# heiheishuang/MuDG

Measured on AMD Instinct MI355X. Metric: DDIM denoise steps/sec, MDM1024 576x1024x16f (CFG: 2 UNet forwards + fused update per step, per clip), higher is better.
Workload: dtype bf16; 1 GPU; MDM1024 latents (B=1,4,16,72,128) + c_concat 8ch, context (B,333,1024), 50-step uniform_trailing DDIM schedule, cfg 7.5, guidance_rescale 0.7, eta 1.0, v-prediction, dynamic rescale; clips_per_gpu=1, parallelism=clip-DP x1 (no in-step collective), launch=hipGraph replay of each UNet pass (cond+uncond batched)

## Files before the change

include/mudg_hip.h:

```cpp
#ifndef MUDG_HIP_H
#define MUDG_HIP_H

#include <stdint.h>

#ifdef __cplusplus
extern "C" {
#endif

#define MUDG_OK          0
#define MUDG_EINVAL     -1
#define MUDG_ELAUNCH    -2
#define MUDG_EUNSUPPORTED -3

int mudg_version(void);
int mudg_operand_dtype(void);
const char* mudg_last_error(void);

typedef struct MudgGemmDesc {
    const void* X;
    const void* X2;
    const void* W;
    void*       Y;
    const float* bias;
    const float* gbias;
// ... 17 lines not shown
    float* stats;
    int subpixel;
    void* Y8; void* S8;
    int ldy8, lds8;
} MudgGemmDesc;
int mudg_gemm(const MudgGemmDesc* d, void* stream);
int mudg_gemm_stats_rows(const MudgGemmDesc* d);
int mudg_conv_subpixel_ok(const MudgGemmDesc* d);

typedef struct MudgAttnDesc {
    const void* Q; const void* K; const void* Vt; void* O;
    int F, heads, Nq, Nk;
    int ldq, ldk, ldvt, ldo;
    int64_t svt;
    int kv_div;
    float scale;
    int accumulate;
    const void* K2; const void* Vt2;
    int Nk2, ldk2, ldvt2, kv_div2;
    int64_t svt2;
    const void* Q8; const void* K8; const void* Qs; const void* Ks;
    int ldq8, ldk8, ldqs, ldks;
    int q_prescaled;
    float* Lse;
} MudgAttnDesc;
int mudg_attention(const MudgAttnDesc* d, void* stream);
int mudg_quantize_mxfp8(const void* X, int ldx, int64_t rows, int cols, void* Y8, int ldy, void* S, int lds, void* stream);

int mudg_temporal_attention(const void* QKV, void* O, int B, int T, int HW, int heads,
                            int ldqkv, int ldo, float scale, void* stream);
int mudg_temporal_self_attention_ok(int T, int HW, int heads, int C, int64_t ldx, int64_t ldw, int64_t ldo);
int mudg_temporal_self_attention(const void* X, const void* Wh, void* O, int B, int T, int HW, int heads, int C, int64_t ldx,
                                 int64_t ldw, int64_t ldo, float scale, void* stream);

int64_t mudg_groupnorm_ws_floats(int samples, int groups, int rows);
int mudg_groupnorm(const void* X, const void* X2, int csplit, int ldx, int ldx2, int x_fp32,
                   const float* gamma, const float* beta, void* Y, int ldy,
                   int samples, int rows, int C, int groups, float eps, int silu,
                   float* ws, void* stream);
int mudg_groupnorm_fused(const void* X, const void* X2, int csplit, int ldx, int ldx2, int x_fp32,
                         const float* gamma, const float* beta, void* Y, int ldy,
                         int samples, int rows, int C, int groups, float eps, int silu,
                         const float* P1, const float* P2, float* ws, void* stream);

int mudg_groupnorm_fused_rows(const void* X, const void* X2, int csplit, int ldx, int ldx2, int x_fp32,
                              const float* gamma, const float* beta, void* Y, int ldy,
                              int samples, int rows, int C, int groups, float eps, int silu,
                              const float* P1, int p1_rows, const float* P2, int p2_rows, float* ws, void* stream);

int mudg_layernorm(const void* X, int ldx, int x_fp32, const float* gamma, const float* beta,
                   void* Y, int ldy, int rows, int C, float eps, void* stream);

int mudg_softmax_rows(const float* S, int lds, void* P, int ldp, int rows, int cols, void* stream);

int mudg_timestep_embedding(const int64_t* t, const float* freqs, float* out, int n, int dim, void* stream);
int mudg_small_linear(const float* x, const void* W, int w_is_bf16, const float* b, float* y,
                      int M, int N, int K, int act_in, int act_out, int accumulate, void* stream);

int mudg_ncthw_to_rows(const void* src, int src_is_fp32, void* dst, int B, int C, int T, int HW,
                       int ld, int coff, int Ttot, int t0, void* stream);
int mudg_rows_to_ncthw(const void* src, int src_is_fp32, int ld, int coff, void* dst, int dst_is_fp32,
                       int B, int C, int T, int HW, float scale, int Ttot, int t0, void* stream);
int mudg_copy_rows(const void* src, int64_t lds, void* dst, int64_t ldd, int64_t rows, int64_t cols, void* stream);
int mudg_axpy_f32(float* y, const float* x, int64_t n, float alpha, void* stream);
int mudg_lincomb(float* out, const float* x, const float* y, const float* ca, const float* cb, int B, int64_t n,
                 void* stream);
// ... 182 lines not shown
```

mudg_amd/csrc/attention.hip:

```cpp
#include "attn_shared.h"
#include <cstdlib>

namespace {

#if MUDG_PLANES == 1
template <bool TWO>
__global__ __launch_bounds__(256, 2) void attn_kernel(const MudgAttnDesc p, const int nqt, const int total) {
    __shared__ __attribute__((aligned(16))) h16 Ks[2 * ATILE];
    __shared__ __attribute__((aligned(16))) h16 Vs[2 * ATILE];

    const int tid = threadIdx.x, lane = tid & 63, wave = tid >> 6;
    const int l31 = lane & 31, hi = lane >> 5;

    const int w = xcd_work_item(total);
    const int pair = w / nqt, qt = w - pair * nqt;
    const int f = pair / p.heads, h = pair - f * p.heads;
    const h16* Qp = reinterpret_cast<const h16*>(p.Q) + (int64_t)f * p.Nq * p.ldq + h * 64;
    h16* Op = reinterpret_cast<h16*>(p.O) + (int64_t)f * p.Nq * p.ldo + h * 64;

    const int q = qt * QB + wave * 32 + l31;
    const bool qok = q < p.Nq;

    h16x8 qf[1][4];
    load_q_frags(qf[0], Qp, q, p.ldq, 0, qok, hi);

    const int lrow = tid >> 3, kc = tid & 7;
    u32x4 kr[1][2], vr[1][2];

    f32x16 o[2], res[TWO ? 2 : 1];
    const float c = p.q_prescaled ? 1.0f : p.scale * 1.4426950408889634f;
    float inv = 0.f;
#pragma unroll
    for (int set = 0; set < (TWO ? 2 : 1); ++set) {
// ... 667 lines not shown
        __syncthreads();
    }

    char* mine = tsa_smem + wave * (2 * 3 * 2048);
#pragma unroll
    for (int pi = 0; pi < 2; ++pi) {
        char* qs = mine + pi * (3 * 2048);
#pragma unroll
        for (int nb = 0; nb < 12; ++nb) {
            Pack8 t;
#pragma unroll
            for (int i = 0; i < 4; ++i) t.h[i] = (h16)acc[pi][nb][i];
            const int u = 4 * (nb & 3) + g;
            const int off = (nb >> 2) == 2 ? c * 128 + ((u ^ tattn_fz(c >> 2)) << 3)
                                           : c * 128 + (((u >> 1) ^ (c & 7)) << 4) + ((u & 1) << 3);
            *reinterpret_cast<u32x2*>(qs + (nb >> 2) * 2048 + off) = t.u;
        }
    }
    __builtin_amdgcn_wave_barrier();
#pragma unroll
    for (int pi = 0; pi < 2; ++pi) {
        const char* qs = mine + pi * (3 * 2048);
        float ov[16];
        tattn_item_mfma(qs, qs + 2048, qs + 4096, c, g, 16, scale, ov);
        h16* dst = O + (row0 + (int64_t)c * HW + (2 * wave + pi)) * ldo + h * 64 + g * 8;
#pragma unroll
        for (int half = 0; half < 2; ++half) {
            h16x8 t;
#pragma unroll
            for (int e = 0; e < 8; ++e) t[e] = (h16)ov[half * 8 + e];
            st16(dst + half * 32, as_u32x4(t));
        }
    }
}
#endif

#if MUDG_PLANES > 1
template <bool TWO>
__global__ __launch_bounds__(256, PLANES == 2 ? 2 : 1) void attn_split_kernel(const MudgAttnDesc p, const int nqt, const int total) {
    extern __shared__ __attribute__((aligned(16))) char smem_raw[];
    h16* Ks = reinterpret_cast<h16*>(smem_raw);
    h16* Vs = Ks + 2 * PLANES * ATILE;

    const int tid = threadIdx.x, lane = tid & 63, wave = tid >> 6;
    const int l31 = lane & 31, hi = lane >> 5;
    const int w = xcd_work_item(total);
    const int pair = w / nqt, qt = w - pair * nqt;
    const int f = pair / p.heads, h = pair - f * p.heads;
    const int psq = p.ldq / PLANES, pso = p.ldo / PLANES;

    const h16* Qp = reinterpret_cast<const h16*>(p.Q) + (int64_t)f * p.Nq * p.ldq + h * 64;
    h16* Op = reinterpret_cast<h16*>(p.O) + (int64_t)f * p.Nq * p.ldo + h * 64;

    const int q = qt * QB + wave * 32 + l31;
    const bool qok = q < p.Nq;
    h16x8 qf[PLANES][4];
#pragma unroll
    for (int pl = 0; pl < PLANES; ++pl) load_q_frags(qf[pl], Qp, q, p.ldq, pl * psq, qok, hi);

    const int lrow = tid >> 3, kc = tid & 7;
    u32x4 kr[PLANES][2], vr[PLANES][2];

    f32x16 o[2], res[TWO ? 2 : 1];
    const float c = p.q_prescaled ? 1.0f : p.scale * 1.4426950408889634f;
#pragma unroll
    for (int set = 0; set < (TWO ? 2 : 1); ++set) {
// ... 575 lines not shown
           ldw >= C && ldo >= C;
#else
    (void)T; (void)HW; (void)heads; (void)C; (void)ldx; (void)ldw; (void)ldo;
    return 0;
#endif
}

extern "C" int mudg_temporal_self_attention(const void* X, const void* Wh, void* O, int B, int T, int HW, int heads, int C, int64_t ldx,
                                            int64_t ldw, int64_t ldo, float scale, void* stream) {
#if MUDG_PLANES == 1
    MUDG_REQUIRE(X && Wh && O, "mudg_temporal_self_attention: null pointer");
    MUDG_REQUIRE(B > 0, "mudg_temporal_self_attention: empty problem");
    MUDG_REQUIRE(aligned16(X) && aligned16(Wh) && aligned16(O), "mudg_temporal_self_attention: alignment");
    if (!mudg_temporal_self_attention_ok(T, HW, heads, C, ldx, ldw, ldo))
        MUDG_FAIL(MUDG_EUNSUPPORTED, "mudg_temporal_self_attention: T=%d HW=%d heads=%d C=%d outside the fused kernel (T = 16, HW %% 8 == 0, "
                  "C = 64 heads, dense 16-byte rows): project with mudg_gemm and call mudg_temporal_attention", T, HW, heads, C);
    const int64_t total = (int64_t)B * (HW / 8) * heads;
    MUDG_REQUIRE(total < (1ll << 31), "mudg_temporal_self_attention: grid too large");
    const int rc0 = mudg_lds_opt_in<tsattn_fused_kernel>(TSA_LDS, "mudg_temporal_self_attention");
    if (rc0 != MUDG_OK) return rc0;
    hipStream_t s = reinterpret_cast<hipStream_t>(stream);
    const int slot = mudg_prof_begin(MUDG_FAM_GEMM, s);
    hipLaunchKernelGGL(tsattn_fused_kernel, dim3((unsigned)total), dim3(256), TSA_LDS, s, (const h16*)X, (const h16*)Wh, (h16*)O, HW, heads, C,
                       ldx, ldw, ldo, scale, (int)total);
    const int rc = mudg_check_launch("mudg_temporal_self_attention");
    const double M = (double)B * T * HW;
    mudg_prof_end(slot, s, 2.0 * M * 3.0 * C * C + 4.0 * (double)B * HW * heads * T * T * 64.0, (2.0 * M * C + 3.0 * C * C) * 2.0);
    return rc;
#else
    (void)X; (void)Wh; (void)O; (void)B; (void)T; (void)HW; (void)heads; (void)C; (void)ldx; (void)ldw; (void)ldo; (void)scale; (void)stream;
    MUDG_FAIL(MUDG_EUNSUPPORTED, "mudg_temporal_self_attention: the fused kernel belongs to the 16-bit operand builds");
#endif
}
```

mudg_amd/csrc/attn_shared.h:

```cpp
#pragma once
#include "common.h"
#include <type_traits>

constexpr int QB = 128;
constexpr int KB = 64;
constexpr int ALD = 72;
constexpr int ATILE = 64 * ALD;

struct KvSet {
    const h16* Kp;
    const h16* Vp;
    int Nk, ldk, ldvt;
    int psk, psv;
};
__device__ __forceinline__ KvSet kv_set(const MudgAttnDesc& p, int f, int h, int set) {
    KvSet kv;
    if (set == 0) {
        kv.Kp = reinterpret_cast<const h16*>(p.K) + (int64_t)(f / p.kv_div) * p.Nk * p.ldk + h * 64;
        kv.Vp = reinterpret_cast<const h16*>(p.Vt) + (int64_t)(f / p.kv_div) * p.svt + (int64_t)(h * 64) * p.ldvt;
        kv.Nk = p.Nk; kv.ldk = p.ldk; kv.ldvt = p.ldvt;
    } else {
        kv.Kp = reinterpret_cast<const h16*>(p.K2) + (int64_t)(f / p.kv_div2) * p.Nk2 * p.ldk2 + h * 64;
        kv.Vp = reinterpret_cast<const h16*>(p.Vt2) + (int64_t)(f / p.kv_div2) * p.svt2 + (int64_t)(h * 64) * p.ldvt2;
        kv.Nk = p.Nk2; kv.ldk = p.ldk2; kv.ldvt = p.ldvt2;
// ... 188 lines not shown
        } else {
#pragma unroll
            for (int r = 0; r < 16; ++r) { o[0][r] = fmaf(o[0][r], inv, res[0][r]); o[1][r] = fmaf(o[1][r], inv, res[1][r]); }
            inv = 1.f;
        }
    }
    return inv;
}
__device__ __forceinline__ void finish_block16(const MudgAttnDesc& p, int f, int h, int q, bool qok, int hi, float c,
                                               float m_run, float l_run, const f32x16 (&o)[2], h16* Op) {
    const float l_tot = l_run + __shfl_xor(l_run, 32, 64);
    const float inv = 1.f / l_tot;
    store_lse(p, f, h, q, qok, hi, c, m_run, l_tot);
    if (qok) store_o16(o, inv, Op + (int64_t)q * p.ldo, hi, p.accumulate);
}

__device__ __forceinline__ __amdgpu_buffer_rsrc_t attn_rsrc(const h16* base) {
    return __builtin_amdgcn_make_buffer_rsrc(const_cast<h16*>(base), 0, (int)0x80000000u, 0x00020000);
}
typedef __attribute__((address_space(3))) void* attn_lptr_t;
__device__ __forceinline__ int swap_mid4(int row) {
    const int i16 = row & 15;
    return (row & ~15) | (i16 & 3) | ((i16 & 8) >> 1) | ((i16 & 4) << 1);
}
__device__ __forceinline__ void dma_offsets(int wave, int lane, int ldk, int ldvt, unsigned (&vk)[2], unsigned (&vv)[2]) {
#pragma unroll
    for (int i = 0; i < 2; ++i) {
        const int row = 16 * wave + 8 * i + (lane >> 3), slot = lane & 7;
        const int chunk = slot ^ ((row >> 1) & 7);
        vk[i] = (unsigned)swap_mid4(row) * (unsigned)ldk * 2u + (unsigned)chunk * 16u;
        vv[i] = (unsigned)row * (unsigned)ldvt * 2u + (unsigned)chunk * 16u;
    }
}
```

mudg_amd/engine/unet.py:

```python
import torch
import torch.nn as nn

from .. import ops
from . import packing as pk



import os as _os
_LEAN_ATTENTION = _os.environ.get("MUDG_ATTN_LEAN", "1") != "0"
_TCONV_SLAB = _os.environ.get("MUDG_TCONV_SLAB", "1") != "0"
_TSATTN_FUSED = _os.environ.get("MUDG_TSATTN_FUSED", "1") != "0"
_FP8_ATTENTION = _os.environ.get("MUDG_ATTN_FP8", "0") == "1"


class _Ctx:
    __slots__ = ("B", "T", "emb", "text", "img", "n_text", "n_img", "img_div", "kv_cache", "replicas", "skips")

    def __init__(self):
        self.replicas, self.skips = 1, None

    def fan_out(self, rows):
        r, self.replicas = self.replicas, 1
        self.B *= r
        self.emb = self.emb.repeat(r, 1)
        if self.skips is not None:
            self.skips[:] = [(ops.repeat_rows(t, r), h, w) for t, h, w in self.skips]
        return ops.repeat_rows(rows, r)


def _gn(mod, x, x2, samples, rows, silu):
    return ops.groupnorm(x, pk.f32(mod, "weight"), pk.f32(mod, "bias"), samples=samples, rows=rows, eps=mod.eps,
                         silu=silu, groups=mod.num_groups, x2=x2)


def _ln(mod, x):
    return ops.layernorm(x, pk.f32(mod, "weight"), pk.f32(mod, "bias"), eps=mod.eps)


def _linear(mod, x, residual=None, x2=None, stream=False, stats=False, hw=0):
    return ops.gemm(x, pk.linear(mod), bias=pk.f32(mod, "bias"), residual=residual, x2=x2, out_stream=stream, stats=stats, frame_rows=hw)


def _conv3x3(mod, x, frames, h, w, *, stride=1, upsample=False, gbias=None, rows_per_group=0, residual=None, x2=None,
             stream=False, stats=True, fp32=False):
    wmat, cpad, korder = pk.conv3x3(mod)
# ... 36 lines not shown
def temporal_conv_block(mod, x, ctx, hw):
    y = x
    stages = (mod.conv1, mod.conv2, mod.conv3, mod.conv4)
    for i, seq in enumerate(stages):
        norm, conv = seq[0], seq[-1]
        y = _gn(norm, y, None, ctx.B, ctx.T * hw, True)
        last = i == len(stages) - 1
        slab = (not last and _TCONV_SLAB and ops.tconv3_slab_ok(ctx.T, hw, conv.weight.shape[1])
                and not ops.tconv3_wide(ctx.T, hw, conv.weight.shape[1], conv.weight.shape[0]))
        y = ops.tconv3(y, pk.tconv(conv, slab), clips=ctx.B, t=ctx.T, hw=hw, cin=conv.weight.shape[1],
                       bias=pk.f32(conv, "bias"), residual=x if last else None, out_stream=last, stats=True, korder=int(slab))
    return y


def res_block(mod, x, x2, h, w, ctx):
    frames, hw = ctx.B * ctx.T, h * w
    a = _gn(mod.in_layers[0], x, x2, frames, hw, True)
    lin = mod.emb_layers[1]
    emb_out = ops.small_linear(ctx.emb, pk.f32(lin, "weight"), pk.f32(lin, "bias"), act_in=True)
    a = _conv3x3(mod.in_layers[2], a, frames, h, w, gbias=emb_out, rows_per_group=ctx.T * hw)
    a = _gn(mod.out_layers[0], a, None, frames, hw, True)
    if isinstance(mod.skip_connection, nn.Identity):
        if x2 is not None:
            raise RuntimeError("identity skip with a concatenated input")
        skip = x
    else:
        skip = _linear(mod.skip_connection, ops.cast_bf16(x), x2=None if x2 is None else ops.cast_bf16(x2), stream=True, hw=hw)
    out = _conv3x3(mod.out_layers[3], a, frames, h, w, residual=skip, stream=True)
    if mod.use_temporal_conv:
        out = temporal_conv_block(mod.temopral_conv, out, ctx, hw)
    return out


def _cross_kv(attn, ctx):
    k_text = ops.gemm(ctx.text, pk.linear(attn.to_k))
    vt_text, ld_text = _vt_projection(attn.to_v, ctx.text, ctx.B, ctx.n_text)
    if ctx.img is None or not attn.image_cross_attention:
        return k_text, vt_text, ld_text, None, None, 0
    k_img = ops.gemm(ctx.img, pk.linear(attn.to_k_ip))
    vt_img, ld_img = _vt_projection(attn.to_v_ip, ctx.img, ctx.img.shape[0] // ctx.n_img, ctx.n_img)
    return k_text, vt_text, ld_text, k_img, vt_img, ld_img


def spatial_block(blk, hcur, frames, hw, ctx, last):
    a1, a2 = blk.attn1, blk.attn2
    c, heads = hcur.shape[1], a1.heads
    n1 = _ln(blk.norm1, hcur)
    lean = _LEAN_ATTENTION and ops.hip.planes() <= 2
    wqk = pk.qk_prescaled(a1, a1.to_q, a1.to_k, a1.scale) if lean else pk.linear_cat(a1, "qk", (a1.to_q, a1.to_k))
    use_fp8 = lean and ops.hip.planes() == 1 and _FP8_ATTENTION and hw >= 512 and hw % 64 == 0
    fp8 = None
    if use_fp8:
        qk, q8, s8 = ops.gemm(n1, wqk, fp8=True)
        fp8 = (q8[:, :c], s8[:, :c // 32], q8[:, c:], s8[:, c // 32:])
    else:
        qk = ops.gemm(n1, wqk, frame_rows=hw)
    vt, ldv = _vt_projection(a1.to_v, n1, frames, hw)
    att = ops.empty_rows(frames * hw, c, ops.H16(), hcur.device)
    ops.attention(qk[:, :c], qk[:, c:], vt, att, frames=frames, heads=heads, nq=hw, nk=hw, ldvt=ldv, svt=c * ldv,
                  scale=a1.scale, q_prescaled=lean, fp8=fp8)
    hcur = _linear(a1.to_out[0], att, residual=hcur, stream=True, hw=hw)
    if ctx.replicas > 1:
        hcur = ctx.fan_out(hcur)
        frames = ctx.B * ctx.T
    n2 = _ln(blk.norm2, hcur)
    q2 = ops.gemm(n2, pk.linear(a2.to_q), frame_rows=hw)
    key = id(a2)
    if key not in ctx.kv_cache:
        ctx.kv_cache[key] = _cross_kv(a2, ctx)
    k_text, vt_text, ld_text, k_img, vt_img, ld_img = ctx.kv_cache[key]
    att2 = ops.empty_rows(frames * hw, c, ops.H16(), hcur.device)
    if k_img is not None and a2.image_cross_attention_scale != 1.0:
        raise NotImplementedError("image_cross_attention_scale != 1.0")
    ops.attention(q2, k_text, vt_text, att2, frames=frames, heads=heads, nq=hw, nk=ctx.n_text, ldvt=ld_text,
                  svt=c * ld_text, kv_div=ctx.T, scale=a2.scale, k2=k_img, vt2=vt_img, nk2=ctx.n_img,
                  ldvt2=ld_img if k_img is not None else None, svt2=c * ld_img if k_img is not None else None,
                  kv_div2=ctx.img_div)
    hcur = _linear(a2.to_out[0], att2, residual=hcur, stream=True, hw=hw)
    return _feed_forward(blk.ff, _ln(blk.norm3, hcur), hcur, stream=not last, hw=hw)


def spatial_transformer(mod, x, h, w, ctx):
    hw = h * w
    cur = _linear(mod.proj_in, _gn(mod.norm, x, None, ctx.B * ctx.T, hw, False), stream=True, hw=hw)
    n = len(mod.transformer_blocks)
    for i, blk in enumerate(mod.transformer_blocks):
        shared = ctx.replicas
        cur = spatial_block(blk, cur, ctx.B * ctx.T, hw, ctx, i == n - 1)
        if ctx.replicas != shared:
            x = ops.repeat_rows(x, shared)
    return _linear(mod.proj_out, cur, residual=x, stream=True, stats=True, hw=hw)


_TSATTN_MAX_C = 640


def _tsattn_fused(t, hw, heads, c, x, out):
    return (_TSATTN_FUSED and c == heads * 64 and c <= _TSATTN_MAX_C
            and ops.temporal_self_attention_ok(t, hw, heads, c, x.stride(0), c, out.stride(0)))


def temporal_block(blk, hcur, hw, ctx, last):
    for attn, norm in ((blk.attn1, blk.norm1), (blk.attn2, blk.norm2)):
        c = hcur.shape[1]
        n = _ln(norm, hcur)
        att = ops.empty_rows(hcur.shape[0], c, ops.H16(), hcur.device)
# ... 240 lines not shown
```

mudg_amd/hip.py:

```python
from __future__ import annotations

import ctypes as C
import os

_HERE = os.path.dirname(os.path.abspath(__file__))
LIB_PATHS = {"bf16": os.path.join(_HERE, "libmudg_hip.so"), "fp16": os.path.join(_HERE, "libmudg_hip_fp16.so"),
             "bf16x3": os.path.join(_HERE, "libmudg_hip_x3.so"), "bf16x6": os.path.join(_HERE, "libmudg_hip_x6.so")}
_MODES = {"bf16": (0, 1), "fp16": (1, 1), "bf16x3": (2, 2), "bf16x6": (3, 3)}
_operand = os.environ.get("MUDG_OPERAND", "bf16").lower()
LIB_PATH = LIB_PATHS["bf16"]


def set_operand(name: str) -> None:
    global _operand
    name = name.lower()
    if name not in LIB_PATHS:
        raise MudgError(f"unknown operand type {name!r} ({' | '.join(LIB_PATHS)})")
    if _lib is not None and name != _operand:
        raise MudgError("the operand type must be chosen before the first kernel call")
    _operand = name


def operand_name() -> str:
    return _operand
# ... 67 lines not shown
class WgradDesc(C.Structure):
    _fields_ = [
        ("A", C.c_void_p), ("B", C.c_void_p), ("out", C.c_void_p),
        ("lda", C.c_int64), ("ldb", C.c_int64), ("P", C.c_int64),
        ("M", C.c_int), ("C", C.c_int), ("taps", C.c_int), ("mode", C.c_int),
        ("Hin", C.c_int), ("Win", C.c_int), ("Hout", C.c_int), ("Wout", C.c_int), ("stride", C.c_int), ("pad", C.c_int),
        ("T", C.c_int), ("HW", C.c_int),
        ("slices", C.c_int), ("chunk", C.c_int64),
    ]


class ShortAttnDesc(C.Structure):
    _fields_ = [
        ("QKV", C.c_void_p), ("O", C.c_void_p),
        ("B", C.c_int), ("heads", C.c_int), ("N", C.c_int), ("d", C.c_int),
        ("ldqkv", C.c_int64), ("ldo", C.c_int64),
        ("scale", C.c_float),
    ]


_P, _I, _L, _F, _D = C.c_void_p, C.c_int, C.c_int64, C.c_float, C.c_double
SIGNATURES = {
    "mudg_version": (_I, []),
    "mudg_operand_dtype": (_I, []),
    "mudg_last_error": (C.c_char_p, []),
    "mudg_gemm": (_I, [C.POINTER(GemmDesc), _P]),
    "mudg_gemm_stats_rows": (_I, [C.POINTER(GemmDesc)]),
    "mudg_conv_subpixel_ok": (_I, [C.POINTER(GemmDesc)]),
    "mudg_attention": (_I, [C.POINTER(AttnDesc), _P]),
    "mudg_quantize_mxfp8": (_I, [_P, _I, _L, _I, _P, _I, _P, _I, _P]),
    "mudg_temporal_attention": (_I, [_P, _P, _I, _I, _I, _I, _I, _I, _F, _P]),
    "mudg_temporal_self_attention_ok": (_I, [_I, _I, _I, _I, _L, _L, _L]),
    "mudg_temporal_self_attention": (_I, [_P, _P, _P, _I, _I, _I, _I, _I, _L, _L, _L, _F, _P]),
    "mudg_groupnorm_ws_floats": (_L, [_I, _I, _I]),
    "mudg_groupnorm": (_I, [_P, _P, _I, _I, _I, _I, _P, _P, _P, _I, _I, _I, _I, _I, _F, _I, _P, _P]),
    "mudg_groupnorm_fused": (_I, [_P, _P, _I, _I, _I, _I, _P, _P, _P, _I, _I, _I, _I, _I, _F, _I, _P, _P, _P, _P]),
    "mudg_groupnorm_fused_rows": (_I, [_P, _P, _I, _I, _I, _I, _P, _P, _P, _I, _I, _I, _I, _I, _F, _I, _P, _I, _P, _I, _P, _P]),
    "mudg_layernorm": (_I, [_P, _I, _I, _P, _P, _P, _I, _I, _I, _F, _P]),
    "mudg_softmax_rows": (_I, [_P, _I, _P, _I, _I, _I, _P]),
    "mudg_timestep_embedding": (_I, [_P, _P, _P, _I, _I, _P]),
    "mudg_small_linear": (_I, [_P, _P, _I, _P, _P, _I, _I, _I, _I, _I, _I, _P]),
    "mudg_ncthw_to_rows": (_I, [_P, _I, _P, _I, _I, _I, _I, _I, _I, _I, _I, _P]),
    "mudg_rows_to_ncthw": (_I, [_P, _I, _I, _I, _P, _I, _I, _I, _I, _I, _F, _I, _I, _P]),
    "mudg_cast_f32_bf16": (_I, [_P, _P, _L, _P]),
    "mudg_cast_rows": (_I, [_P, _I, _L, _P, _I, _L, _L, _L, _P]),
    "mudg_zero_channels": (_I, [_P, _I, _I, _I, _I, _P]),
    "mudg_copy_rows": (_I, [_P, _L, _P, _L, _L, _L, _P]),
    "mudg_axpy_f32": (_I, [_P, _P, _L, _F, _P]),
    "mudg_lincomb": (_I, [_P, _P, _P, _P, _P, _I, _L, _P]),
    "mudg_ddim_ws_doubles": (_L, [_I]),
    "mudg_frames_to_u8": (_I, [_P, _P, _I, _I, _I, _L, _P]),
    "mudg_log_sheet": (_I, [_P, _P, _I, _I, _I, _I, _I, _I, _I, _P]),
    "mudg_depth_from_u8": (_I, [_P, _P, _L, _P]),
    "mudg_semantic_nearest": (_I, [_P, _P, _P, _L, _P]),
    "mudg_splat_points": (_I, [_P, _P, _L, _P, _I, _I, _P, _I, _I, _F, _F, _F, _F, _F, _F, _F, _I, _P, _P]),
    "mudg_splat_resolve": (_I, [_P, _P, _L, _P, _P, _L, _P]),
    "mudg_splat_compose": (_I, [_P, _P, _P, _P, _P, _P, _L, _I, _I, _I, _I, _I, _P, _P, _P, _P]),
    "mudg_cloud_sweep": (_I, [_P, _P, _P, _P, _I, _L, _L, _P, _P, _I, _P, _I, _P, _L, _P, _P, _P]),
    "mudg_cloud_voxel_keys": (_I, [_P, _L, _D, _P, _P]),
    "mudg_cloud_voxel_reduce": (_I, [_P, _P, _P, _L, _D, _P, _L, _P]),
    "mudg_cloud_voxel_finish": (_I, [_P, _L, _D, _P, _P]),
    "mudg_depth_align_sums": (_I, [_P, _P, _I, _I, _I, _P, _P]),
    "mudg_depth_align_solve": (_I, [_P, _I, _P, _P, _P]),
    "mudg_depth_finish": (_I, [_P, _P, _P, _L, _I, _I, _I, _P, _P, _P]),
    "mudg_colormap_spectral": (_I, [_P, _L, _D, _D, _I, _P, _P, _P]),
    "mudg_depth_unproject": (_I, [_P, _P, _P, _L, _P, _I, _I, _I, _D, _D, _P, _P, _P]),
# ... 119 lines not shown
```

mudg_amd/ops.py:

```python
from __future__ import annotations

import ctypes as C
import math
from typing import Optional

import torch

from . import hip



def H16():
    return hip.operand_dtype()


def STREAM():
    import os
    if hip.operand_name() != "bf16" or os.environ.get("MUDG_STREAM", "").lower() == "fp32":
        return torch.float32
    return torch.float16


def kind(t) -> int:
    if t.dtype == torch.float32:
# ... 247 lines not shown
    rows, cols = x.shape
    y = torch.empty((rows, cols), dtype=torch.uint8, device=x.device)
    sc = torch.empty((rows, cols // 32), dtype=torch.uint8, device=x.device)
    hip.check(hip.lib().mudg_quantize_mxfp8(x.data_ptr(), x.stride(0), rows, cols, y.data_ptr(), y.stride(0), sc.data_ptr(),
                                            sc.stride(0), _stream()), "mudg_quantize_mxfp8")
    return y, sc


def temporal_attention(qkv, out, *, clips, t, hw, heads, scale=0.125):
    hip.check(hip.lib().mudg_temporal_attention(qkv.data_ptr(), out.data_ptr(), clips, t, hw, heads,
                                                qkv.stride(0), out.stride(0), scale, _stream()),
              "mudg_temporal_attention")
    return out


def temporal_self_attention_ok(t, hw, heads, c, ldx=None, ldw=None, ldo=None):
    return bool(hip.lib().mudg_temporal_self_attention_ok(t, hw, heads, c, c if ldx is None else ldx, c if ldw is None else ldw,
                                                          c if ldo is None else ldo))


def temporal_self_attention(x, wh, out, *, clips, t, hw, heads, scale=0.125):
    _rows(x); _rows(wh); _rows(out)
    rows, c = x.shape
    if rows != clips * t * hw or tuple(out.shape) != (rows, c) or tuple(wh.shape) != (3 * c, c):
        raise hip.MudgError(f"temporal_self_attention: x {tuple(x.shape)}, wh {tuple(wh.shape)}, out {tuple(out.shape)} are not "
                            f"[clips * t * hw = {clips * t * hw}][C], [3C][C], [clips * t * hw][C]")
    _drop_stats(out)
    hip.check(hip.lib().mudg_temporal_self_attention(x.data_ptr(), wh.data_ptr(), out.data_ptr(), clips, t, hw, heads, x.shape[1],
                                                     x.stride(0), wh.stride(0), out.stride(0), scale, _stream()),
              "mudg_temporal_self_attention")
    return out


def _rows_any(t):
    if t.dim() != 2 or t.stride(1) != 1 or t.dtype not in (H16(), torch.float32, torch.float16) or not t.is_cuda:
        raise hip.MudgError(f"expected a cuda operand / fp32 / fp16 rows matrix, got {tuple(t.shape)} {t.dtype} on {t.device}")
    return t


def groupnorm(x, gamma, beta, *, samples, rows, eps, silu, groups=32, x2=None, out=None, fused=True, return_stats=False):
    _rows_any(x)
    if x2 is not None and x2.dtype != x.dtype:
        raise hip.MudgError("groupnorm: both channel sources must share a dtype")
    c = x.shape[1] + (x2.shape[1] if x2 is not None else 0)
    if out is None:
        out = empty_rows(samples * rows, c, H16(), x.device)
    def partials(t):
        ws = getattr(t, GN_ATTR, None)
        tiled = getattr(t, GN_ATTR + "_clips", 0)
        if tiled and tiled != samples:
            return None, 128
        ok_ = ws is not None and getattr(t, GN_ATTR + "_version", -1) == _version(t)
        return (ws if ok_ else None), getattr(t, GN_ATTR + "_rows", 128)

    p1, r1 = partials(x) if fused else (None, 128)
    p2, r2 = partials(x2) if (fused and x2 is not None) else (None, r1)
    ok = p1 is not None and rows % r1 == 0 and p1.shape[1] == x.shape[1] and p1.shape[0] * r1 >= samples * rows
    if ok and x2 is not None:
        ok = p2 is not None and rows % r2 == 0 and p2.shape[1] == x2.shape[1] and p2.shape[0] * r2 >= samples * rows
    if ok:
        ws = torch.empty(2 * samples * groups, dtype=torch.float32, device=x.device)
        hip.check(hip.lib().mudg_groupnorm_fused_rows(x.data_ptr(), _ptr(x2), x.shape[1], x.stride(0),
                                                      x2.stride(0) if x2 is not None else 0, kind(x),
                                                      gamma.data_ptr(), beta.data_ptr(),
                                                      out.data_ptr(), out.stride(0), samples, rows, c, groups, eps, int(silu),
                                                      p1.data_ptr(), r1, _ptr(p2), r2, ws.data_ptr(), _stream()), "mudg_groupnorm_fused")
# ... 848 lines not shown
```

Measured before the change: 8.716 steps/s.

## Fold Q and output projections into cross-attention K/V and fuse LN

Adds a folded cross-attention kernel. Wq is pre-multiplied into the text and image keys, and Wo into the values, once per conditioning. The new kernel then computes the scores straight from the (optionally layer-normalised) hidden rows and writes the output projection plus bias and residual in one pass. This removes the LayerNorm, Q-projection GEMM, attention and out-projection launches, along with their intermediate HBM traffic, for blocks with C<=320. In exchange it does C-wide instead of 64-wide dot products per head and stores the folded K/V in reduced precision, which changes numerics.

```diff
diff --git a/include/mudg_hip.h b/include/mudg_hip.h
--- a/include/mudg_hip.h
+++ b/include/mudg_hip.h
@@ -73,6 +73,12 @@
 int mudg_temporal_self_attention_ok(int T, int HW, int heads, int C, int64_t ldx, int64_t ldw, int64_t ldo);
 int mudg_temporal_self_attention(const void* X, const void* Wh, void* O, int B, int T, int HW, int heads, int C, int64_t ldx,
                                  int64_t ldw, int64_t ldo, float scale, void* stream);
+
+int mudg_cross_attention_folded_ok(int HW, int heads, int C, int n_text, int n_img, int64_t ldx, int64_t ldr, int64_t ldo);
+int mudg_cross_attention_folded(const void* X, int64_t ldx, int x_kind, const float* gamma, const float* beta, float eps,
+                                const void* R, int64_t ldr, const void* Kt, const void* Vt, const void* Ki, const void* Vi,
+                                const float* bias, void* O, int64_t ldo, int stream_kind, int frames, int HW, int heads, int C,
+                                int n_text, int n_img, int kv_div, int kv_div2, void* stream);
 
 int64_t mudg_groupnorm_ws_floats(int samples, int groups, int rows);
 int mudg_groupnorm(const void* X, const void* X2, int csplit, int ldx, int ldx2, int x_fp32,
diff --git a/mudg_amd/csrc/attention.hip b/mudg_amd/csrc/attention.hip
--- a/mudg_amd/csrc/attention.hip
+++ b/mudg_amd/csrc/attention.hip
@@ -1,4 +1,5 @@
 #include "attn_shared.h"
+#include "gemm_shared.h"
 #include <cstdlib>
 
 namespace {
@@ -732,6 +733,236 @@
             st16(dst + half * 32, as_u32x4(t));
         }
     }
+}
+
+struct XfoldArgs {
+    const void* X; const void* R; void* O;
+    const h16 *Kt, *Vt, *Ki, *Vi;
+    const float *gamma, *beta, *bias;
+    int64_t ldx, ldr, ldo;
+    int HW, n_text, n_img, kv_div, kv_div2, total;
+    float eps;
+};
+
+template <int NH, int RB, bool LN, int SK>
+__global__ __launch_bounds__(256, NH * RB <= 5 ? 2 : 1) void xfold_kernel(const XfoldArgs a) {
+    constexpr int C = NH * 64, TILE = 64 * RB, NKS = C / 32, NB = C / 16;
+    extern __shared__ __attribute__((aligned(16))) char xf_smem[];
+    const int tid = threadIdx.x, lane = tid & 63, wave = tid >> 6;
+    const int c = lane & 15, g = lane >> 4;
+    const int tile = xcd_work_item(a.total);
+    const int64_t row0 = (int64_t)tile * TILE;
+    const int f = (int)(row0 / a.HW);
+    const int64_t wrow = row0 + wave * (16 * RB);
+    const bool img = a.n_img > 0;
+    const h16* ktext = a.Kt + (int64_t)(f / a.kv_div) * NH * XF_TEXT * C;
+    const h16* vtext = a.Vt + (int64_t)(f / a.kv_div) * NH * C * XF_TEXT;
+    const h16* kimg = img ? a.Ki + (int64_t)(f / a.kv_div2) * NH * XF_IMG * C : nullptr;
+    const h16* vimg = img ? a.Vi + (int64_t)(f / a.kv_div2) * NH * C * XF_IMG : nullptr;
+
+    char* xw = xf_smem + XF_LDS + wave * (RB * NKS * 1024) + lane * 16;
+    if constexpr (!LN) {
+#pragma unroll
+        for (int rb = 0; rb < RB; ++rb)
+#pragma unroll
+            for (int ks = 0; ks < NKS; ++ks)
+                st16(xw + (rb * NKS + ks) * 1024, ld16(reinterpret_cast<const h16*>(a.X) + (wrow + rb * 16 + c) * a.ldx + ks * 32 + g * 8));
+    } else {
+#pragma unroll
+        for (int rb = 0; rb < RB; ++rb) {
+            float x[NKS][8];
+            float s = 0.f;
+#pragma unroll
+            for (int ks = 0; ks < NKS; ++ks) {
+                load_piece8(a.X, SK, (wrow + rb * 16 + c) * a.ldx + ks * 32 + g * 8, 0, x[ks]);
+#pragma unroll
+                for (int e = 0; e < 8; ++e) s += x[ks][e];
+            }
+            s += __shfl_xor(s, 16, 64); s += __shfl_xor(s, 32, 64);
+            const float mean = s / (float)C;
+            float q = 0.f;
+#pragma unroll
+            for (int ks = 0; ks < NKS; ++ks)
+#pragma unroll
+                for (int e = 0; e < 8; ++e) { const float d = x[ks][e] - mean; q = fmaf(d, d, q); }
+            q += __shfl_xor(q, 16, 64); q += __shfl_xor(q, 32, 64);
+            const float rstd = rsqrtf(q / (float)C + a.eps);
+#pragma unroll
+            for (int ks = 0; ks < NKS; ++ks) {
+                float gm[8], bt[8];
+                load_piece8(a.gamma, KIND_F32, ks * 32 + g * 8, 0, gm);
+                load_piece8(a.beta, KIND_F32, ks * 32 + g * 8, 0, bt);
+                h16x8 o;
+#pragma unroll
+                for (int e = 0; e < 8; ++e) o[e] = (h16)fmaf((x[ks][e] - mean) * rstd, gm[e], bt[e]);
+                st16(xw + (rb * NKS + ks) * 1024, as_u32x4(o));
+            }
+            __builtin_amdgcn_sched_barrier(0);
+        }
+    }
+
+    const int lrow = tid >> 3, lch = tid & 7;
+    const bool k2_text = lrow < 16;
+    const int koff2 = (k2_text ? 64 + lrow : lrow - 16) * C + lch * 8;
+    const int klds = lrow * 128 + ((lch ^ (lrow & 7)) << 4);
+    const bool v2_text = tid < 128;
+    int voff[3], vlds[3], vkey[3];
+#pragma unroll
+    for (int i = 0; i < 3; ++i) {
+        const int p = tid + 256 * i;
+        const bool text = i < 2 || v2_text;
+        const int vrow = text ? p / 10 : (p - 640) >> 1;
+        const int vch = text ? p - vrow * 10 : 10 + (p & 1);
+        voff[i] = text ? vrow * XF_TEXT + vch * 8 : vrow * XF_IMG + (vch - 10) * 8;
+        vlds[i] = vrow * XF_VLD + vch * 16;
+        vkey[i] = text ? vch * 8 : (vch - 10) * 8;
+    }
+    const int vlim2 = v2_text ? a.n_text : a.n_img;
+
+    u32x4 nx[2][3];
+    auto fetch = [&](int h, int j) {
+        u32x4 (&n)[3] = nx[j & 1];
+        if (j >= 2 * NH) { j -= 2 * NH; ++h; }
+        if (h >= NH) return;
+        if (j < NH) {
+            const h16* kt = ktext + (int64_t)h * XF_TEXT * C + j * 64;
+            n[0] = ld16(kt + lrow * C + lch * 8);
+            n[1] = ld16(kt + (lrow + 32) * C + lch * 8);
+            if (k2_text) n[2] = ld16(kt + koff2);
+            else n[2] = img ? ld16(kimg + (int64_t)h * XF_IMG * C + j * 64 + koff2) : zero16();
+        } else {
+            const int vc = j - NH;
+            const h16* vt = vtext + ((int64_t)h * C + vc * 64) * XF_TEXT;
+            n[0] = ld16(vt + voff[0]);
+            n[1] = ld16(vt + voff[1]);
+            if (v2_text) n[2] = ld16(vt + voff[2]);
+            else n[2] = img ? ld16(vimg + ((int64_t)h * C + vc * 64) * XF_IMG + voff[2]) : zero16();
+        }
+    };
+    auto stage = [&](int h, int j) {
+        const u32x4 (&n)[3] = nx[j & 1];
+        char* st = xf_smem + (j & 1) * XF_STAGE;
+        if (j >= 2 * NH) { j -= 2 * NH; ++h; }
+        if (h >= NH) return;
+        if (j < NH) {
+#pragma unroll
+            for (int i = 0; i < 3; ++i) st16(st + klds + 4096 * i, n[i]);
+        } else {
+            st16(st + vlds[0], xf_zero_pad(n[0], vkey[0], a.n_text));
+            st16(st + vlds[1], xf_zero_pad(n[1], vkey[1], a.n_text));
+            st16(st + vlds[2], xf_zero_pad(n[2], vkey[2], vlim2));
+        }
+    };
+
+    f32x4 acc[RB][NB];
+#pragma unroll
+    for (int rb = 0; rb < RB; ++rb)
+#pragma unroll
+        for (int nb = 0; nb < NB; ++nb) acc[rb][nb] = f32x4{0.f, 0.f, 0.f, 0.f};
+
+    fetch(0, 0);
+    fetch(0, 1);
+    stage(0, 0);
+    __syncthreads();
+    for (int h = 0; h < NH; ++h) {
+        f32x4 s[RB][6];
+#pragma unroll
+        for (int rb = 0; rb < RB; ++rb)
+#pragma unroll
+            for (int kb = 0; kb < 6; ++kb) s[rb][kb] = f32x4{0.f, 0.f, 0.f, 0.f};
+#pragma unroll
+        for (int kc = 0; kc < NH; ++kc) {
+            const char* cur = xf_smem + (kc & 1) * XF_STAGE;
+            fetch(h, kc + 2);
+#pragma unroll
+            for (int s2 = 0; s2 < 2; ++s2) {
+                const int foff = c * 128 + (((g + 4 * s2) ^ (c & 7)) << 4);
+                h16x8 xf[RB];
+#pragma unroll
+                for (int rb = 0; rb < RB; ++rb) xf[rb] = as_h16x8(ld16(xw + (rb * NKS + 2 * kc + s2) * 1024));
+#pragma unroll
+                for (int kb = 0; kb < 6; ++kb) {
+                    const h16x8 kf = as_h16x8(ld16(cur + kb * 2048 + foff));
+#pragma unroll
+                    for (int rb = 0; rb < RB; ++rb) s[rb][kb] = MFMA_16x16x32(kf, xf[rb], s[rb][kb]);
+                }
+            }
+            stage(h, kc + 1);
+            __syncthreads();
+        }
+
+        h16x8 pt[RB][2];
+        mf4 pl[RB], pi[RB];
+        float inv_t[RB], inv_i[RB];
+#pragma unroll
+        for (int rb = 0; rb < RB; ++rb) {
+            h16 p[24];
+            inv_t[rb] = xf_softmax<5>(&s[rb][0], a.n_text, g, &p[0]);
+            inv_i[rb] = img ? xf_softmax<1>(&s[rb][5], a.n_img, g, &p[20]) : 0.f;
+            union { mf4 m; h16 e[4]; } ul, ui;
+#pragma unroll
+            for (int i = 0; i < 4; ++i) {
+                pt[rb][0][i] = p[i]; pt[rb][0][4 + i] = p[4 + i];
+                pt[rb][1][i] = p[8 + i]; pt[rb][1][4 + i] = p[12 + i];
+                ul.e[i] = p[16 + i];
+                ui.e[i] = img ? p[20 + i] : (h16)0.f;
+            }
+            pl[rb] = ul.m; pi[rb] = ui.m;
+            asm volatile("" : "+v"(inv_t[rb]), "+v"(inv_i[rb]));
+        }
+
+#pragma unroll
+        for (int vc = 0; vc < NH; ++vc) {
+            const char* cur = xf_smem + ((NH + vc) & 1) * XF_STAGE;
+            fetch(h, NH + vc + 2);
+#pragma unroll
+            for (int nb = 0; nb < 4; ++nb) {
+                const char* vr = cur + (16 * nb + c) * XF_VLD;
+                const h16x8 v0 = as_h16x8(ld16(vr + 16 * g)), v1 = as_h16x8(ld16(vr + 64 + 16 * g));
+                const mf4 vl = *reinterpret_cast<const mf4*>(vr + 128 + 8 * g), vi = *reinterpret_cast<const mf4*>(vr + 160 + 8 * g);
+#pragma unroll
+                for (int rb = 0; rb < RB; ++rb) {
+                    f32x4 t = {0.f, 0.f, 0.f, 0.f}, tl = {0.f, 0.f, 0.f, 0.f}, u = {0.f, 0.f, 0.f, 0.f};
+                    t = MFMA_16x16x32(v0, pt[rb][0], t);
+                    tl = MFMA_16x16x16(vl, pl[rb], tl);
+                    u = MFMA_16x16x16(vi, pi[rb], u);
+                    t = MFMA_16x16x32(v1, pt[rb][1], t);
+                    float r[4];
+#pragma unroll
+                    for (int i = 0; i < 4; ++i) r[i] = fmaf(u[i], inv_i[rb], fmaf(t[i] + tl[i], inv_t[rb], acc[rb][4 * vc + nb][i]));
+                    asm volatile("" : "+v"(r[0]), "+v"(r[1]), "+v"(r[2]), "+v"(r[3]));
+                    acc[rb][4 * vc + nb] = f32x4{r[0], r[1], r[2], r[3]};
+                }
+            }
+            stage(h, NH + vc + 1);
+            __syncthreads();
+        }
+    }
+
+    float* ep = reinterpret_cast<float*>(xf_smem) + wave * (16 * XF_ELD);
+    const int er = lane >> 3, ec = (lane & 7) * 8;
+#pragma unroll
+    for (int rb = 0; rb < RB; ++rb)
+#pragma unroll
+        for (int q = 0; q < NH; ++q) {
+#pragma unroll
+            for (int nb = 0; nb < 4; ++nb) *reinterpret_cast<f32x4*>(ep + c * XF_ELD + 16 * nb + 4 * g) = acc[rb][4 * q + nb];
+            __builtin_amdgcn_wave_barrier();
+#pragma unroll
+            for (int j = 0; j < 2; ++j) {
+                const int r = er + 8 * j, col = 64 * q + ec;
+                const f32x4 lo = *reinterpret_cast<const f32x4*>(ep + r * XF_ELD + ec), hi = *reinterpret_cast<const f32x4*>(ep + r * XF_ELD + ec + 4);
+                float v[8], bs[8];
+                load_piece8(a.bias, KIND_F32, col, 0, bs);
+#pragma unroll
+                for (int e = 0; e < 4; ++e) { v[e] = lo[e] + bs[e]; v[4 + e] = hi[e] + bs[4 + e]; }
+                const int64_t row = wrow + rb * 16 + r;
+                add_residual(v, a.R, SK, row * a.ldr + col, 0, 8, true);
+                store_piece<8>(a.O, row * a.ldo + col, SK, 0, v, 8, true);
+            }
+            __builtin_amdgcn_wave_barrier();
+            __builtin_amdgcn_sched_barrier(0);
+        }
 }
 #endif
 
@@ -1373,3 +1604,80 @@
     MUDG_FAIL(MUDG_EUNSUPPORTED, "mudg_temporal_self_attention: the fused kernel belongs to the 16-bit operand builds");
 #endif
 }
+
+extern "C" int mudg_cross_attention_folded_ok(int HW, int heads, int C, int n_text, int n_img, int64_t ldx, int64_t ldr, int64_t ldo) {
+#if MUDG_PLANES == 1
+    if (!(heads == 1 || heads == 2 || heads == 4 || heads == 5 || heads == 10) || C != heads * 64) return 0;
+    const int tile = 64;
+    const bool ok = HW > 0 && HW % tile == 0 && n_text >= 64 && n_text <= XF_TEXT && n_img >= 0 && n_img <= XF_IMG && ldx % 8 == 0 &&
+                    ldr % 8 == 0 && ldo % 8 == 0 && ldx >= C && ldr >= C && ldo >= C;
+    return ok ? tile : 0;
+#else
+    (void)HW; (void)heads; (void)C; (void)n_text; (void)n_img; (void)ldx; (void)ldr; (void)ldo;
+    return 0;
+#endif
+}
+
+extern "C" int mudg_cross_attention_folded(const void* X, int64_t ldx, int x_kind, const float* gamma, const float* beta, float eps,
+                                           const void* R, int64_t ldr, const void* Kt, const void* Vt, const void* Ki, const void* Vi,
+                                           const float* bias, void* O, int64_t ldo, int stream_kind, int frames, int HW, int heads,
+                                           int C, int n_text, int n_img, int kv_div, int kv_div2, void* stream) {
+#if MUDG_PLANES == 1
+    MUDG_REQUIRE(X && R && O && Kt && Vt && bias, "mudg_cross_attention_folded: null pointer");
+    MUDG_REQUIRE((gamma == nullptr) == (beta == nullptr), "mudg_cross_attention_folded: gamma and beta come together");
+    MUDG_REQUIRE(frames > 0 && kv_div > 0 && kv_div2 > 0, "mudg_cross_attention_folded: empty problem");
+    MUDG_REQUIRE(n_img == 0 || (Ki && Vi), "mudg_cross_attention_folded: image keys without their operands");
+    MUDG_REQUIRE(stream_kind == KIND_F16 || stream_kind == KIND_F32, "mudg_cross_attention_folded: the stream rows are fp16 (2) or fp32 (1)");
+    MUDG_REQUIRE(x_kind == (gamma ? stream_kind : KIND_OPERAND),
+                 "mudg_cross_attention_folded: X is the normalised operand rows, or with gamma / beta the stream rows");
+    MUDG_REQUIRE(aligned16(X) && aligned16(R) && aligned16(O) && aligned16(Kt) && aligned16(Vt) && aligned16(Ki) && aligned16(Vi) &&
+                 aligned16(bias) && aligned16(gamma) && aligned16(beta), "mudg_cross_attention_folded: alignment");
+    const int tile = mudg_cross_attention_folded_ok(HW, heads, C, n_text, n_img, ldx, ldr, ldo);
+    if (!tile)
+        MUDG_FAIL(MUDG_EUNSUPPORTED, "mudg_cross_attention_folded: HW=%d heads=%d C=%d n_text=%d n_img=%d outside the folded kernel (HW whole "
+                  "tiles of 64 rows; C = 64 heads in {64, 128, 256, 320, 640}; 64 <= n_text <= 80; n_img <= 16; dense 16-byte "
+                  "rows): project with mudg_gemm and call mudg_attention", HW, heads, C, n_text, n_img);
+    const int64_t total = (int64_t)frames * HW / tile;
+    MUDG_REQUIRE(total < (1ll << 31), "mudg_cross_attention_folded: grid too large");
+    XfoldArgs a;
+    a.X = X; a.R = R; a.O = O;
+    a.Kt = (const h16*)Kt; a.Vt = (const h16*)Vt; a.Ki = (const h16*)Ki; a.Vi = (const h16*)Vi;
+    a.gamma = gamma; a.beta = beta; a.bias = bias;
+    a.ldx = ldx; a.ldr = ldr; a.ldo = ldo;
+    a.HW = HW; a.n_text = n_text; a.n_img = n_img; a.kv_div = kv_div; a.kv_div2 = kv_div2;
+    a.total = (int)total; a.eps = eps;
+    hipStream_t s = reinterpret_cast<hipStream_t>(stream);
+    const int slot = mudg_prof_begin(MUDG_FAM_ATTN, s);
+    int rc_lds = MUDG_OK;
+    auto launch = [&](auto nh, auto rb) {
+        constexpr int NH = decltype(nh)::value, RB = decltype(rb)::value;
+        constexpr int lds = XF_LDS + 4 * RB * (NH * 2) * 1024;
+        if ((rc_lds = mudg_lds_opt_in<&xfold_kernel<NH, RB, true, KIND_F16>>(lds, "mudg_cross_attention_folded")) != MUDG_OK) return;
+        if ((rc_lds = mudg_lds_opt_in<&xfold_kernel<NH, RB, true, KIND_F32>>(lds, "mudg_cross_attention_folded")) != MUDG_OK) return;
+        if ((rc_lds = mudg_lds_opt_in<&xfold_kernel<NH, RB, false, KIND_F16>>(lds, "mudg_cross_attention_folded")) != MUDG_OK) return;
+        if ((rc_lds = mudg_lds_opt_in<&xfold_kernel<NH, RB, false, KIND_F32>>(lds, "mudg_cross_attention_folded")) != MUDG_OK) return;
+        if (gamma && stream_kind == KIND_F16) hipLaunchKernelGGL((xfold_kernel<NH, RB, true, KIND_F16>), dim3((unsigned)total), dim3(256), lds, s, a);
+        else if (gamma) hipLaunchKernelGGL((xfold_kernel<NH, RB, true, KIND_F32>), dim3((unsigned)total), dim3(256), lds, s, a);
+        else if (stream_kind == KIND_F16) hipLaunchKernelGGL((xfold_kernel<NH, RB, false, KIND_F16>), dim3((unsigned)total), dim3(256), lds, s, a);
+        else hipLaunchKernelGGL((xfold_kernel<NH, RB, false, KIND_F32>), dim3((unsigned)total), dim3(256), lds, s, a);
+    };
+    using one = std::integral_constant<int, 1>;
+    switch (heads) {
+        case 1: launch(std::integral_constant<int, 1>{}, one{}); break;
+        case 2: launch(std::integral_constant<int, 2>{}, one{}); break;
+        case 4: launch(std::integral_constant<int, 4>{}, one{}); break;
+        case 5: launch(std::integral_constant<int, 5>{}, one{}); break;
+        default: launch(std::integral_constant<int, 10>{}, one{}); break;
+    }
+    if (rc_lds != MUDG_OK) return rc_lds;
+    const int rc = mudg_check_launch("mudg_cross_attention_folded");
+    const double M = (double)frames * HW;
+    mudg_prof_end(slot, s, 4.0 * M * heads * 96.0 * C, M * C * (gamma ? 4.0 : 6.0));
+    return rc;
+#else
+    (void)X; (void)ldx; (void)x_kind; (void)gamma; (void)beta; (void)eps; (void)R; (void)ldr; (void)Kt; (void)Vt; (void)Ki; (void)Vi;
+    (void)bias; (void)O; (void)ldo; (void)stream_kind; (void)frames; (void)HW; (void)heads; (void)C; (void)n_text; (void)n_img; (void)kv_div;
+    (void)kv_div2; (void)stream;
+    MUDG_FAIL(MUDG_EUNSUPPORTED, "mudg_cross_attention_folded: the folded kernel belongs to the 16-bit operand builds");
+#endif
+}
diff --git a/mudg_amd/csrc/attn_shared.h b/mudg_amd/csrc/attn_shared.h
--- a/mudg_amd/csrc/attn_shared.h
+++ b/mudg_amd/csrc/attn_shared.h
@@ -244,3 +244,47 @@
         vv[i] = (unsigned)row * (unsigned)ldvt * 2u + (unsigned)chunk * 16u;
     }
 }
+
+constexpr int XF_TEXT = 80, XF_IMG = 16;
+constexpr int XF_VLD = 208;
+constexpr int XF_STAGE = 64 * XF_VLD;
+static_assert(XF_STAGE >= 96 * 128, "a stage holds a K' chunk");
+constexpr int XF_LDS = 2 * XF_STAGE;
+constexpr int XF_ELD = 68;
+static_assert(XF_LDS >= 4 * 16 * XF_ELD * 4, "the dead stages hold the four waves' epilogue patches");
+
+__device__ __forceinline__ u32x4 xf_zero_pad(u32x4 v, int key0, int n) {
+    if (key0 + 8 > n) {
+        h16x8 hv = as_h16x8(v);
+#pragma unroll
+        for (int e = 0; e < 8; ++e) if (key0 + e >= n) hv[e] = (h16)0.f;
+        v = as_u32x4(hv);
+    }
+    return v;
+}
+template <int NBK>
+__device__ __forceinline__ float xf_softmax(const f32x4* s, int n, int g, h16* p) {
+    float v[NBK][4];
+    float mx = -INFINITY;
+#pragma unroll
+    for (int kb = 0; kb < NBK; ++kb)
+#pragma unroll
+        for (int i = 0; i < 4; ++i) {
+            v[kb][i] = (16 * kb + 4 * g + i < n) ? s[kb][i] : -INFINITY;
+            mx = fmaxf(mx, v[kb][i]);
+        }
+    mx = fmaxf(mx, __shfl_xor(mx, 16, 64));
+    mx = fmaxf(mx, __shfl_xor(mx, 32, 64));
+    float l = 0.f;
+#pragma unroll
+    for (int kb = 0; kb < NBK; ++kb)
+#pragma unroll
+        for (int i = 0; i < 4; ++i) {
+            const h16 r = (h16)__builtin_amdgcn_exp2f(v[kb][i] - mx);
+            p[4 * kb + i] = r;
+            l += (float)r;
+        }
+    l += __shfl_xor(l, 16, 64);
+    l += __shfl_xor(l, 32, 64);
+    return 1.f / l;
+}
diff --git a/mudg_amd/engine/unet.py b/mudg_amd/engine/unet.py
--- a/mudg_amd/engine/unet.py
+++ b/mudg_amd/engine/unet.py
@@ -11,6 +11,7 @@
 _TCONV_SLAB = _os.environ.get("MUDG_TCONV_SLAB", "1") != "0"
 _TSATTN_FUSED = _os.environ.get("MUDG_TSATTN_FUSED", "1") != "0"
 _FP8_ATTENTION = _os.environ.get("MUDG_ATTN_FP8", "0") == "1"
+_XATTN_FOLDED = _os.environ.get("MUDG_XATTN_FOLDED", "1") != "0"
 
 
 class _Ctx:
@@ -113,14 +114,65 @@
     return out
 
 
+_XF_TEXT, _XF_IMG = 80, 16
+_XATTN_MAX_C = 320
+_XF_SLOTS = {}
+_XATTN_NORM_INSIDE_MAX_C = 320
+
+
+def _xattn_folded(c, heads, n_text, n_img, hw, ldx=None, ldo=None):
+    return bool(_XATTN_FOLDED and c == heads * 64 and c <= _XATTN_MAX_C
+                and ops.cross_attention_folded_ok(hw, heads, c, n_text, n_img, ldx, ldx, ldo))
+
+
+def _xf_text_slots(device):
+    hit = _XF_SLOTS.get(device)
+    if hit is None:
+        idx = list(range(_XF_TEXT))
+        for s in range(64):
+            ks, r = divmod(s, 32)
+            g, e = divmod(r, 8)
+            idx[s] = 32 * ks + 16 * (e >> 2) + 4 * g + (e & 3)
+        hit = _XF_SLOTS[device] = torch.tensor(idx, dtype=torch.int64, device=device)
+    return hit
+
+
+def _fold_kv(attn, to_k, to_v, tokens, batches, n, slots):
+    import math
+    heads = attn.heads
+    wq = attn.to_q.weight.detach().float()
+    wo = attn.to_out[0].weight.detach().float()
+    c = wq.shape[1]
+    tok = tokens.float()
+    k = (tok @ to_k.weight.detach().float().t()).reshape(batches, n, heads, 64)
+    v = (tok @ to_v.weight.detach().float().t()).reshape(batches, n, heads, 64)
+    kf = torch.einsum("bjhd,hdc->bhjc", k, wq.reshape(heads, 64, c)) * (float(attn.scale) * math.log2(math.e))
+    vf = torch.einsum("bjhd,chd->bhjc", v, wo.reshape(c, heads, 64))
+    pad = (0, 0, 0, slots - n)
+    kf = torch.nn.functional.pad(kf, pad).to(ops.H16()).contiguous()
+    vf = torch.nn.functional.pad(vf, pad).to(ops.H16())
+    if slots == _XF_TEXT:
+        vf = vf.index_select(2, _xf_text_slots(vf.device))
+    return kf, vf.transpose(2, 3).contiguous()
+
+
 def _cross_kv(attn, ctx):
     k_text = ops.gemm(ctx.text, pk.linear(attn.to_k))
     vt_text, ld_text = _vt_projection(attn.to_v, ctx.text, ctx.B, ctx.n_text)
-    if ctx.img is None or not attn.image_cross_attention:
-        return k_text, vt_text, ld_text, None, None, 0
+    with_img = ctx.img is not None and attn.image_cross_attention
+    c = attn.to_q.weight.shape[1]
+    folded = (None, None, None, None)
+    if tuple(attn.to_q.weight.shape) == (c, c) and _xattn_folded(c, attn.heads, ctx.n_text, ctx.n_img if with_img else 0, 128):
+        folded = _fold_kv(attn, attn.to_k, attn.to_v, ctx.text, ctx.B, ctx.n_text, _XF_TEXT)
+        if with_img:
+            folded += _fold_kv(attn, attn.to_k_ip, attn.to_v_ip, ctx.img, ctx.img.shape[0] // ctx.n_img, ctx.n_img, _XF_IMG)
+        else:
+            folded += (None, None)
+    if not with_img:
+        return (k_text, vt_text, ld_text, None, None, 0) + folded
     k_img = ops.gemm(ctx.img, pk.linear(attn.to_k_ip))
     vt_img, ld_img = _vt_projection(attn.to_v_ip, ctx.img, ctx.img.shape[0] // ctx.n_img, ctx.n_img)
-    return k_text, vt_text, ld_text, k_img, vt_img, ld_img
+    return (k_text, vt_text, ld_text, k_img, vt_img, ld_img) + folded
 
 
 def spatial_block(blk, hcur, frames, hw, ctx, last):
@@ -144,15 +196,24 @@
     if ctx.replicas > 1:
         hcur = ctx.fan_out(hcur)
         frames = ctx.B * ctx.T
-    n2 = _ln(blk.norm2, hcur)
-    q2 = ops.gemm(n2, pk.linear(a2.to_q), frame_rows=hw)
     key = id(a2)
     if key not in ctx.kv_cache:
         ctx.kv_cache[key] = _cross_kv(a2, ctx)
-    k_text, vt_text, ld_text, k_img, vt_img, ld_img = ctx.kv_cache[key]
-    att2 = ops.empty_rows(frames * hw, c, ops.H16(), hcur.device)
+    k_text, vt_text, ld_text, k_img, vt_img, ld_img, kf_text, vf_text, kf_img, vf_img = ctx.kv_cache[key]
     if k_img is not None and a2.image_cross_attention_scale != 1.0:
         raise NotImplementedError("image_cross_attention_scale != 1.0")
+    n_img = ctx.n_img if k_img is not None else 0
+    if kf_text is not None and ops.kind(hcur) != 0 and _xattn_folded(c, heads, ctx.n_text, n_img, hw, hcur.stride(0), c):
+        out = ops.empty_rows(frames * hw, c, ops.STREAM(), hcur.device)
+        inside = c <= _XATTN_NORM_INSIDE_MAX_C
+        norm = (pk.f32(blk.norm2, "weight"), pk.f32(blk.norm2, "bias"), blk.norm2.eps) if inside else None
+        hcur = ops.cross_attention_folded(hcur if inside else _ln(blk.norm2, hcur), hcur, out, kf_text, vf_text, kf_img, vf_img,
+                                          pk.f32(a2.to_out[0], "bias"), frames=frames, hw=hw, heads=heads, n_text=ctx.n_text, n_img=n_img,
+                                          kv_div=ctx.T, kv_div2=ctx.img_div, norm=norm)
+        return _feed_forward(blk.ff, _ln(blk.norm3, hcur), hcur, stream=not last, hw=hw)
+    n2 = _ln(blk.norm2, hcur)
+    q2 = ops.gemm(n2, pk.linear(a2.to_q), frame_rows=hw)
+    att2 = ops.empty_rows(frames * hw, c, ops.H16(), hcur.device)
     ops.attention(q2, k_text, vt_text, att2, frames=frames, heads=heads, nq=hw, nk=ctx.n_text, ldvt=ld_text,
                   svt=c * ld_text, kv_div=ctx.T, scale=a2.scale, k2=k_img, vt2=vt_img, nk2=ctx.n_img,
                   ldvt2=ld_img if k_img is not None else None, svt2=c * ld_img if k_img is not None else None,
diff --git a/mudg_amd/hip.py b/mudg_amd/hip.py
--- a/mudg_amd/hip.py
+++ b/mudg_amd/hip.py
@@ -123,6 +123,8 @@
     "mudg_temporal_attention": (_I, [_P, _P, _I, _I, _I, _I, _I, _I, _F, _P]),
     "mudg_temporal_self_attention_ok": (_I, [_I, _I, _I, _I, _L, _L, _L]),
     "mudg_temporal_self_attention": (_I, [_P, _P, _P, _I, _I, _I, _I, _I, _L, _L, _L, _F, _P]),
+    "mudg_cross_attention_folded_ok": (_I, [_I, _I, _I, _I, _I, _L, _L, _L]),
+    "mudg_cross_attention_folded": (_I, [_P, _L, _I, _P, _P, _F, _P, _L, _P, _P, _P, _P, _P, _P, _L, _I, _I, _I, _I, _I, _I, _I, _I, _I, _P]),
     "mudg_groupnorm_ws_floats": (_L, [_I, _I, _I]),
     "mudg_groupnorm": (_I, [_P, _P, _I, _I, _I, _I, _P, _P, _P, _I, _I, _I, _I, _I, _F, _I, _P, _P]),
     "mudg_groupnorm_fused": (_I, [_P, _P, _I, _I, _I, _I, _P, _P, _P, _I, _I, _I, _I, _I, _F, _I, _P, _P, _P, _P]),
diff --git a/mudg_amd/ops.py b/mudg_amd/ops.py
--- a/mudg_amd/ops.py
+++ b/mudg_amd/ops.py
@@ -303,6 +303,36 @@
     return out
 
 
+def cross_attention_folded_ok(hw, heads, c, n_text, n_img, ldx=None, ldr=None, ldo=None):
+    return hip.lib().mudg_cross_attention_folded_ok(hw, heads, c, n_text, n_img, c if ldx is None else ldx, c if ldr is None else ldr,
+                                                    c if ldo is None else ldo)
+
+
+def cross_attention_folded(x, residual, out, kt, vt, ki, vi, bias, *, frames, hw, heads, n_text, n_img, kv_div=1, kv_div2=1, norm=None):
+    _rows(x) if norm is None else _rows_any(x)
+    _rows_any(residual); _rows_any(out)
+    rows, c = out.shape
+    if rows != frames * hw or tuple(x.shape) != (rows, c) or tuple(residual.shape) != (rows, c) or c != heads * 64:
+        raise hip.MudgError(f"cross_attention_folded: x {tuple(x.shape)}, residual {tuple(residual.shape)}, out {tuple(out.shape)} are "
+                            f"not [frames * hw = {frames * hw}][64 heads = {heads * 64}]")
+    if kind(residual) != kind(out) or (norm is not None and kind(x) != kind(out)):
+        raise hip.MudgError("cross_attention_folded: the stream rows (residual, out, and x when it is normalised here) share one storage kind")
+    clips, imgs = -(-frames // kv_div), -(-frames // kv_div2)
+    need = [(kt, clips * heads * 80 * c), (vt, clips * heads * c * 80)]
+    if n_img:
+        need += [(ki, imgs * heads * 16 * c), (vi, imgs * heads * c * 16)]
+    for t, n in need:
+        if t is None or t.dtype != H16() or not t.is_cuda or not t.is_contiguous() or t.numel() < n:
+            raise hip.MudgError("cross_attention_folded: a folded operand is missing, not dense operand data, or too small for the frames")
+    _drop_stats(out)
+    gamma, beta, eps = norm if norm is not None else (None, None, 0.0)
+    hip.check(hip.lib().mudg_cross_attention_folded(
+        x.data_ptr(), x.stride(0), kind(x), _ptr(gamma), _ptr(beta), eps, residual.data_ptr(), residual.stride(0), kt.data_ptr(),
+        vt.data_ptr(), _ptr(ki) if n_img else None, _ptr(vi) if n_img else None, bias.data_ptr(), out.data_ptr(), out.stride(0), kind(out),
+        frames, hw, heads, c, n_text, n_img, kv_div, kv_div2, _stream()), "mudg_cross_attention_folded")
+    return out
+
+
 def _rows_any(t):
     if t.dim() != 2 or t.stride(1) != 1 or t.dtype not in (H16(), torch.float32, torch.float16) or not t.is_cuda:
         raise hip.MudgError(f"expected a cuda operand / fp32 / fp16 rows matrix, got {tuple(t.shape)} {t.dtype} on {t.device}")
```

Result: no change. 8.713 steps/s (-0.0%).
